# cvg/LightGlue

Hardware: AMD Instinct MI355X
Metric: image-pairs/s at N=M=1024, 9 layers; match-index parity vs ref (higher is better)
Workload: dtype f16; 1 GPU; SuperPoint-dim 256-d descriptors, N=M=1024, 9 layers, pruning/early-stop OFF, batch=32 pairs per GPU, seeded random weights (recipe A), precision=f16x3 (split-f16 operands, 3 MFMAs per product, for every contraction incl. q k^T and P V; fp32 accumulate / residual / softmax); pairs_per_gpu=32, keypoints=1024, keypoints1=1024, descriptor_dim=256, parallelism=pair-sharded dp1, batches_in_flight=1

## Files before the change

lightglue_amd/csrc/lg_assign.hip:

```cpp
#include "lg_kernels.h"

namespace lg {

__device__ __forceinline__ float fexp(float x) { return __builtin_amdgcn_exp2f(x * 1.44269504088896340736f); }

__device__ __forceinline__ void lse_merge(float& m, float& s, float m2, float s2) {
    const float mn = fmaxf(m, m2);
    if (mn == -INFINITY) { m = mn; s = 0.f; return; }
    s = s * fexp(m - mn) + s2 * fexp(m2 - mn);
    m = mn;
}

constexpr int ART = 32;

__device__ __forceinline__ void lse_merge1(float& m, float& s, float m2, float s2) {
    const float e = (m == m2) ? 1.f : fexp(-fabsf(m - m2));
    const bool keep = m >= m2;
    s = keep ? __builtin_fmaf(s2, e, s) : __builtin_fmaf(s, e, s2);
    m = keep ? m : m2;
}

__global__ __launch_bounds__(256) void lse_sweep_kernel(AssignArgs a) {
    const int pair = blockIdx.y, tile = blockIdx.x, tid = threadIdx.x, lane = tid & 63, wave = tid >> 6;
    const int len0 = a.rs.len[2 * pair], len1 = a.rs.len[2 * pair + 1];
    const int r0 = tile * ART;
    if (r0 >= len0) return;
    const int rows = min(ART, len0 - r0);
    const int ntiles = a.rs.cap0 / ART;
    const float* simp = a.sim + ((long long)pair * a.rs.cap0 + r0) * a.rs.cap1;
    float* pm = a.cpm + ((long long)pair * ntiles + tile) * a.rs.cap1;
    float* ps = a.cps + ((long long)pair * ntiles + tile) * a.rs.cap1;
    __shared__ float shm[4][ART], shs[4][ART];
    for (int c0 = 0; c0 < len1; c0 += 1024) {
        const int c = c0 + tid * 4;
        const bool act = c < len1;
        const float* col = simp + (act ? c : 0);
        float cm[4] = {-INFINITY, -INFINITY, -INFINITY, -INFINITY}, cs[4] = {0.f, 0.f, 0.f, 0.f};
        f32x4 nxt = *reinterpret_cast<const f32x4*>(col);
#pragma unroll 1
        for (int r = 0; r < rows; ++r) {
            f32x4 v = nxt;
            nxt = *reinterpret_cast<const f32x4*>(col + (long long)min(r + 1, rows - 1) * a.rs.cap1);
#pragma unroll
            for (int i = 0; i < 4; ++i) if (!act || c + i >= len1) v[i] = -INFINITY;
            const float m = wave_allmax(fmaxf(fmaxf(v[0], v[1]), fmaxf(v[2], v[3])));
            float sum = 0.f;
            if (m != -INFINITY) sum = (fexp(v[0] - m) + fexp(v[1] - m)) + (fexp(v[2] - m) + fexp(v[3] - m));
            if (act) {
#pragma unroll
                for (int i = 0; i < 4; ++i) lse_merge1(cm[i], cs[i], v[i], v[i] == -INFINITY ? 0.f : 1.f);
            }
            sum = wave_allsum(sum);
            if (lane == 0) {
                if (c0 == 0) { shm[wave][r] = m; shs[wave][r] = sum; }
                else { float mo = shm[wave][r], so = shs[wave][r]; lse_merge1(mo, so, m, sum); shm[wave][r] = mo; shs[wave][r] = so; }
            }
        }
        if (act) {
            *reinterpret_cast<f32x4*>(pm + c) = f32x4{cm[0], cm[1], cm[2], cm[3]};
            *reinterpret_cast<f32x4*>(ps + c) = f32x4{cs[0], cs[1], cs[2], cs[3]};
        }
    }
    __syncthreads();
    if (tid < rows) {
        float m = shm[0][tid], s = shs[0][tid];
        for (int w = 1; w < 4; ++w) lse_merge1(m, s, shm[w][tid], shs[w][tid]);
        a.lse_r[(long long)pair * a.rs.cap0 + r0 + tid] = m + logf(s);
    }
}

__global__ __launch_bounds__(256) void col_lse_merge_kernel(AssignArgs a) {
    const int pair = blockIdx.y, lane = threadIdx.x & 63, wave = threadIdx.x >> 6, c = blockIdx.x * 64 + lane;
    const int len0 = a.rs.len[2 * pair], len1 = a.rs.len[2 * pair + 1];
    if (blockIdx.x * 64 >= len1) return;
    const int ntiles = a.rs.cap0 / ART, live = (len0 + ART - 1) / ART;
    const int cc = min(c, a.rs.cap1 - 1);
    const float* pm = a.cpm + (long long)pair * ntiles * a.rs.cap1 + cc;
    const float* ps = a.cps + (long long)pair * ntiles * a.rs.cap1 + cc;
    float m = -INFINITY, s = 0.f;
#pragma unroll 8
    for (int t = wave; t < live; t += 4) lse_merge1(m, s, pm[(long long)t * a.rs.cap1], ps[(long long)t * a.rs.cap1]);
    __shared__ float shm[4][64], shs[4][64];
    shm[wave][lane] = m; shs[wave][lane] = s;
    __syncthreads();
    if (wave == 0 && c < len1) {
#pragma unroll
        for (int w = 1; w < 4; ++w) lse_merge1(m, s, shm[w][lane], shs[w][lane]);
        a.lse_c[(long long)pair * a.rs.cap1 + c] = m + logf(s);
    }
}

__device__ __forceinline__ float score_of(float sim, float lr, float lc, float cert) {
    return ((sim - lr) + (sim - lc)) + cert;
}

__global__ __launch_bounds__(256) void argmax_sweep_kernel(AssignArgs a) {
    const int pair = blockIdx.y, tile = blockIdx.x, tid = threadIdx.x, lane = tid & 63, wave = tid >> 6;
    const int len0 = a.rs.len[2 * pair], len1 = a.rs.len[2 * pair + 1];
    const int r0 = tile * ART;
    if (r0 >= len0) return;
    const int rows = min(ART, len0 - r0);
    const int ntiles = a.rs.cap0 / ART;
    const float* simp = a.sim + ((long long)pair * a.rs.cap0 + r0) * a.rs.cap1;
    const float* lsec = a.lse_c + (long long)pair * a.rs.cap1;
    const float* ls1 = a.ls + seg_row_base(a.rs, 2 * pair + 1);
    const float* lser = a.lse_r + (long long)pair * a.rs.cap0 + r0;
    const float* ls0 = a.ls + seg_row_base(a.rs, 2 * pair) + r0;
    float* pv = a.cbv + ((long long)pair * ntiles + tile) * a.rs.cap1;
    int* pi = a.cbi + ((long long)pair * ntiles + tile) * a.rs.cap1;
    __shared__ float shb[4][ART]; __shared__ int shi[4][ART];
    for (int c0 = 0; c0 < len1; c0 += 1024) {
        const int c = c0 + tid * 4;
        const bool act = c < len1;
        const int cc = act ? c : 0;
        const float* col = simp + cc;
        const f32x4 lc = *reinterpret_cast<const f32x4*>(lsec + cc);
        const f32x4 l1 = *reinterpret_cast<const f32x4*>(ls1 + cc);
        float cb[4] = {-INFINITY, -INFINITY, -INFINITY, -INFINITY}; int ci[4] = {0, 0, 0, 0};
        f32x4 nxt = *reinterpret_cast<const f32x4*>(col);
#pragma unroll 1
        for (int r = 0; r < rows; ++r) {
            const f32x4 v = nxt;
            nxt = *reinterpret_cast<const f32x4*>(col + (long long)min(r + 1, rows - 1) * a.rs.cap1);
            const float lr = lser[r], l0 = ls0[r];
            float best = -INFINITY; int bi = 0x7fffffff;
#pragma unroll
            for (int i = 0; i < 4; ++i) {
                if (act && c + i < len1) {
                    const float sc = score_of(v[i], lr, lc[i], l0 + l1[i]);
                    if (sc > best) { best = sc; bi = c + i; }
                    if (sc > cb[i]) { cb[i] = sc; ci[i] = r0 + r; }
                }
            }
            const float wbest = wave_allmax(best);
            const unsigned long long owners = __ballot(best == wbest);
            const int wbi = __builtin_amdgcn_readlane(bi, (int)__builtin_ctzll(owners));
            if (lane == 0) {
                if (c0 == 0 || wbest > shb[wave][r]) { shb[wave][r] = wbest; shi[wave][r] = wbi; }
            }
        }
        if (act) {
            *reinterpret_cast<f32x4*>(pv + c) = f32x4{cb[0], cb[1], cb[2], cb[3]};
            *reinterpret_cast<int4*>(pi + c) = int4{ci[0], ci[1], ci[2], ci[3]};
        }
    }
    __syncthreads();
    if (tid < rows) {
        float best = shb[0][tid]; int bi = shi[0][tid];
        for (int w = 1; w < 4; ++w) {
            const float ob = shb[w][tid]; const int oi = shi[w][tid];
            if (ob > best || (ob == best && oi < bi)) { best = ob; bi = oi; }
        }
        a.max0[(long long)pair * a.rs.cap0 + r0 + tid] = best; a.arg0[(long long)pair * a.rs.cap0 + r0 + tid] = bi;
    }
}

__global__ __launch_bounds__(256) void col_argmax_merge_kernel(AssignArgs a) {
    const int pair = blockIdx.y, lane = threadIdx.x & 63, wave = threadIdx.x >> 6, c = blockIdx.x * 64 + lane;
    const int len0 = a.rs.len[2 * pair], len1 = a.rs.len[2 * pair + 1];
    if (blockIdx.x * 64 >= len1) return;
    const int ntiles = a.rs.cap0 / ART, live = (len0 + ART - 1) / ART;
    const int cc = min(c, a.rs.cap1 - 1);
    const float* pv = a.cbv + (long long)pair * ntiles * a.rs.cap1 + cc;
    const int* pi = a.cbi + (long long)pair * ntiles * a.rs.cap1 + cc;
    float best = -INFINITY; int bi = 0;
#pragma unroll 8
    for (int t = wave; t < live; t += 4) {
        const float v = pv[(long long)t * a.rs.cap1];
        const int vi = pi[(long long)t * a.rs.cap1];
        if (v > best) { best = v; bi = vi; }
    }
    __shared__ float shb[4][64]; __shared__ int shi[4][64];
    shb[wave][lane] = best; shi[wave][lane] = bi;
    __syncthreads();
    if (wave == 0 && c < len1) {
#pragma unroll
        for (int w = 1; w < 4; ++w) {
            const float v = shb[w][lane]; const int vi = shi[w][lane];
            if (v > best || (v == best && v != -INFINITY && vi < bi)) { best = v; bi = vi; }
        }
        a.max1[(long long)pair * a.rs.cap1 + c] = best; a.arg1[(long long)pair * a.rs.cap1 + c] = bi;
    }
}

struct Row0 { bool valid; int j; float e; };
__device__ __forceinline__ Row0 match_of_row0(const AssignArgs& a, const float* max0, const int* arg0, const int* arg1, int r, int len1) {
    const int jraw = arg0[r];
    const bool jok = (unsigned)jraw < (unsigned)len1;
    const int j = jok ? jraw : 0;
    const bool mutual0 = jok && arg1[j] == r;
    const float e = mutual0 ? expf(max0[r]) : 0.f;
    return {mutual0 && (e > a.filter_threshold), j, e};
}
__global__ __launch_bounds__(256) void finalize_kernel(AssignArgs a) {
    const int pair = blockIdx.y, blk = blockIdx.x, tid = threadIdx.x, lane = tid & 63, wave = tid >> 6;
    const int len0 = a.rs.len[2 * pair], len1 = a.rs.len[2 * pair + 1];
    const int base0 = seg_row_base(a.rs, 2 * pair), base1 = seg_row_base(a.rs, 2 * pair + 1);
    const float* max0 = a.max0 + (long long)pair * a.rs.cap0;
    const int* arg0 = a.arg0 + (long long)pair * a.rs.cap0;
    const int* arg1 = a.arg1 + (long long)pair * a.rs.cap1;
    int* m0 = a.m0 + (long long)pair * a.n0; float* s0 = a.s0 + (long long)pair * a.n0;
    int* m1 = a.m1 + (long long)pair * a.n1; float* s1 = a.s1 + (long long)pair * a.n1;
    __shared__ int sh_cnt[4], sh_below[4];
    if (len0 == 0 || len1 == 0) { if (blk == 0 && tid == 0) a.n_matches[pair] = 0; return; }
    {
        const int b = blk * 256 + tid;
        if (b < len1) {
            const int i = arg1[b];
            const bool mutual1 = arg0[i] == b;
            const float e = expf(max0[i]);
            const bool valid1 = mutual1 && (e > a.filter_threshold);
            const int ob = a.ind[base1 + b];
            m1[ob] = valid1 ? a.ind[base0 + i] : -1;
            s1[ob] = mutual1 ? e : 0.f;
        }
    }
    if (blk * 256 >= len0 && blk != (int)gridDim.x - 1) return;
    int below = 0;
    for (int q = 0; q < blk; ++q) {
        const int r = q * 256 + tid;
        below += __popcll(__ballot(r < len0 && match_of_row0(a, max0, arg0, arg1, min(r, len0 - 1), len1).valid));
    }
    const int r = blk * 256 + tid;
    bool valid0 = false; int oa = 0, ob = -1; float e = 0.f;
    if (r < len0) {
        const Row0 m = match_of_row0(a, max0, arg0, arg1, r, len1);
        valid0 = m.valid; e = m.e;
        oa = a.ind[base0 + r];
        ob = valid0 ? a.ind[base1 + m.j] : -1;
        m0[oa] = ob;
        s0[oa] = e;
    }
    const unsigned long long bal = __ballot(valid0);
    const int prefix = __popcll(bal & ((1ull << lane) - 1ull));
    if (lane == 0) { sh_cnt[wave] = __popcll(bal); sh_below[wave] = below; }
    __syncthreads();
    int woff = sh_below[0] + sh_below[1] + sh_below[2] + sh_below[3];
    for (int w = 0; w < wave; ++w) woff += sh_cnt[w];
    if (valid0) {
        int* ml = a.matches + (long long)pair * a.max_matches * 2;
        float* msl = a.mscores + (long long)pair * a.max_matches;
        const int k = woff + prefix;
        ml[2 * k] = oa; ml[2 * k + 1] = ob; msl[k] = e;
    }
    if (blk == (int)gridDim.x - 1 && tid == 0)
        a.n_matches[pair] = sh_below[0] + sh_below[1] + sh_below[2] + sh_below[3] + sh_cnt[0] + sh_cnt[1] + sh_cnt[2] + sh_cnt[3];
}

__global__ __launch_bounds__(256) void fill_neg_inf_kernel(float* p, long long n) {
    for (long long i = (long long)blockIdx.x * 256 + threadIdx.x; i < n; i += (long long)gridDim.x * 256) p[i] = -INFINITY;
}
__global__ __launch_bounds__(256) void log_assignment_kernel(AssignArgs a) {
    const int pair = blockIdx.y, r = blockIdx.x, tid = threadIdx.x;
    const int len0 = a.rs.len[2 * pair], len1 = a.rs.len[2 * pair + 1];
    const int base0 = seg_row_base(a.rs, 2 * pair), base1 = seg_row_base(a.rs, 2 * pair + 1);
    float* out = a.log_assignment + (long long)pair * (a.n0 + 1) * (a.n1 + 1);
    if (len0 == 0 || len1 == 0) {
        if (r == a.rs.cap0 && tid == 0) out[(long long)a.n0 * (a.n1 + 1) + a.n1] = 0.f;
        return;
    }
    if (r == a.rs.cap0) {
        for (int c = tid; c < len1; c += 256) out[(long long)a.n0 * (a.n1 + 1) + a.ind[base1 + c]] = a.lsneg[base1 + c];
        if (tid == 0) out[(long long)a.n0 * (a.n1 + 1) + a.n1] = 0.f;
        return;
    }
    if (r >= len0) return;
    float* orow = out + (long long)a.ind[base0 + r] * (a.n1 + 1);
    const float* simr = a.sim + ((long long)pair * a.rs.cap0 + r) * a.rs.cap1;
    const float lr = a.lse_r[(long long)pair * a.rs.cap0 + r], l0 = a.ls[base0 + r];
    const float* lsec = a.lse_c + (long long)pair * a.rs.cap1;
    for (int c = tid; c < len1; c += 256) orow[a.ind[base1 + c]] = score_of(simr[c], lr, lsec[c], l0 + a.ls[base1 + c]);
    if (tid == 0) orow[a.n1] = a.lsneg[base0 + r];
}

hipError_t launch_assign(const AssignArgs& a, hipStream_t s) {
    const int B = a.rs.B;
    hipError_t e;
    if (!a.all_rows_live) {
    if (a.n0 > 0) {
        if ((e = hipMemsetAsync(a.m0, 0xFF, sizeof(int) * (size_t)B * a.n0, s)) != hipSuccess) return e;
        if ((e = hipMemsetAsync(a.s0, 0, sizeof(float) * (size_t)B * a.n0, s)) != hipSuccess) return e;
    }
    if (a.n1 > 0) {
        if ((e = hipMemsetAsync(a.m1, 0xFF, sizeof(int) * (size_t)B * a.n1, s)) != hipSuccess) return e;
        if ((e = hipMemsetAsync(a.s1, 0, sizeof(float) * (size_t)B * a.n1, s)) != hipSuccess) return e;
    }
    }
    hipLaunchKernelGGL(lse_sweep_kernel, dim3(a.rs.cap0 / ART, B), dim3(256), 0, s, a);
    hipLaunchKernelGGL(col_lse_merge_kernel, dim3(a.rs.cap1 / 64, B), dim3(256), 0, s, a);
    hipLaunchKernelGGL(argmax_sweep_kernel, dim3(a.rs.cap0 / ART, B), dim3(256), 0, s, a);
    hipLaunchKernelGGL(col_argmax_merge_kernel, dim3(a.rs.cap1 / 64, B), dim3(256), 0, s, a);
    hipLaunchKernelGGL(finalize_kernel, dim3((max(a.rs.cap0, a.rs.cap1) + 255) / 256, B), dim3(256), 0, s, a);
    if (a.log_assignment) {
        const long long total = (long long)B * (a.n0 + 1) * (a.n1 + 1);
        hipLaunchKernelGGL(fill_neg_inf_kernel, dim3(2048), dim3(256), 0, s, a.log_assignment, total);
        hipLaunchKernelGGL(log_assignment_kernel, dim3(a.rs.cap0 + 1, B), dim3(256), 0, s, a);
    }
    return hipGetLastError();
}

}
```

lightglue_amd/csrc/lg_proj.hip:

```cpp
#include "lg_proj_body.h"
#include "lg_side.h"

namespace lg {

__device__ __forceinline__ bool proj_tile(const RowSpace& rs, TileLoc& t, int& len) {
    t = locate_tile(rs, blockIdx.x, PBM);
    len = rs.len[t.seg];
    if (t.r0 >= len) return false;
    if (rs.active && !rs.active[t.pair]) return false;
    return true;
}
__device__ __forceinline__ bool proj_tile(const RowSpace& rs, TileLoc& t) { int len; return proj_tile(rs, t, len); }

template <int PREC> struct TileRegs {
    static constexpr int NV = PJ<PREC>::Tag::EPC / 4, KE = PJL<PREC>::KE, STAGES = PJL<PREC>::STAGES;
    f32x4 v[STAGES][NV];
    __device__ __forceinline__ void load(const float* src) {
#pragma unroll
        for (int st = 0; st < STAGES; ++st)
#pragma unroll
            for (int j = 0; j < NV; ++j) v[st][j] = *reinterpret_cast<const f32x4*>(src + st * KE + 4 * j);
    }
    __device__ __forceinline__ void load_f16(const f16_t* src) {
#pragma unroll
        for (int st = 0; st < STAGES; ++st) {
            if constexpr (NV == 2) {
                const f16x8 h = *reinterpret_cast<const f16x8*>(src + st * KE);
                v[st][0] = widen4_f16(h.lo); v[st][1] = widen4_f16(h.hi);
            } else {
                static_assert(NV == 1, "4 or 8 elements per chunk");
                v[st][0] = widen4_f16(*reinterpret_cast<const f16x4*>(src + st * KE));
            }
        }
    }
    __device__ __forceinline__ void store(char* smA, int srow, int sslot, bool copy_out, float* xdst) const {
        const int off = pj_tile_off(srow, sslot);
#pragma unroll
        for (int st = 0; st < STAGES; ++st) {
            if (copy_out) {
#pragma unroll
                for (int j = 0; j < NV; ++j) *reinterpret_cast<f32x4*>(xdst + st * KE + 4 * j) = v[st][j];
            }
            char* tile = smA + st * PJL<PREC>::TILE;
            if constexpr (PREC == PREC_F32) {
                *reinterpret_cast<f32x4*>(tile + off) = v[st][0];
            } else if constexpr (PJ<PREC>::APART == 2) {
                u32x4 hi, lo;
                split8<typename PJ<PREC>::Tag>(v[st][0], v[st][1], hi, lo);
                *reinterpret_cast<u32x4*>(tile + off) = hi;
                *reinterpret_cast<u32x4*>(tile + PJL<PREC>::A_PLANE + off) = lo;
            } else {
                *reinterpret_cast<u32x4*>(tile + off) = pack8<typename PJ<PREC>::Tag>(v[st][0], v[st][1]);
            }
        }
    }
};
template <int PREC>
__device__ __forceinline__ void proj_load_tile(const float* X, const TileLoc& t, char* smA) {
    const int srow = threadIdx.x >> 3, sslot = threadIdx.x & 7;
    TileRegs<PREC> h;
    h.load(X + (long long)(t.grow0 + srow) * 256 + sslot * PJ<PREC>::Tag::EPC);
    h.store(smA, srow, sslot, false, nullptr);
}

template <int PREC, class TA, int NTP, int NPASS>
__global__ __launch_bounds__(PTHREADS) void proj_kernel(ProjArgs a) {
    extern __shared__ __attribute__((aligned(16))) char smem[];
    char* smA = smem;

    TileLoc t;
    if (!proj_tile(a.rs, t)) return;
    const int tid = threadIdx.x, lane = tid & 63, w = __builtin_amdgcn_readfirstlane(tid >> 6);
    if (a.dbg && lane == 0) dbg_slot(a.dbg, w, 0) = clock64();
    RopeRows<4> rr;
    if constexpr (NTP == 3) proj_rope_load<4>(a, t, rr);
    proj_load_tile<PREC>(a.X, t, smA);
    proj_compute<PREC, TA, NTP, NPASS>(a, t, smA, 0, NTP == 3 ? &rr : nullptr);
}

struct RowDest { float* X; float* cosb; float* sinb; };

struct FirstRows {
    typedef PrepArgs Args;
    const PrepArgs& pa;
    const PrepSide& sd;
    int seg; long long simg, in_row;
    __device__ __forceinline__ FirstRows(const PrepArgs& pa_, const TileLoc& t, int rc) : pa(pa_), sd(pa_.side[t.seg & 1]), seg(t.seg) {
        simg = source_image(pa.px, t.pair, seg & 1);
        in_row = simg * sd.n + rc;
    }
    template <int PREC> __device__ __forceinline__ void load_x(TileRegs<PREC>& h, int col) const {
        if (sd.kind == DESC_F16) h.load_f16(static_cast<const f16_t*>(sd.desc) + in_row * 256 + col);
        else h.load(static_cast<const float*>(sd.desc) + in_row * 256 + col);
    }
    __device__ __forceinline__ void rotary(int sslot, f32x4& c4, f32x4& s4) const {
        float kn[4];
        normalised_keypoint(pa, sd, seg, simg, in_row, kn);
#pragma unroll
        for (int f = 0; f < 4; ++f) {
            const float p = fourier_phase(pa, kn, sslot * 4 + f);
            c4[f] = cosf(p); s4[f] = sinf(p);
        }
    }
    __device__ __forceinline__ RowDest dest() const { return {pa.X, pa.cosb, pa.sinb}; }
    __device__ __forceinline__ void row_stored(long long grow, int r, int sslot) const { if (sslot == 0) pa.ind[grow] = r; }
};
struct GatherRows {
    typedef GatherArgs Args;
    const GatherArgs& ga;
    long long in_row;
    __device__ __forceinline__ GatherRows(const GatherArgs& ga_, const TileLoc& t, int rc) : ga(ga_) {
        const long long base = t.grow0 - t.r0;
        const int sr = ga.len_old[t.seg] >= 0 ? ga.src[base + rc] : rc;
        in_row = base + sr;
    }
    template <int PREC> __device__ __forceinline__ void load_x(TileRegs<PREC>& h, int col) const { h.load(ga.Xold + in_row * 256 + col); }
    __device__ __forceinline__ void rotary(int sslot, f32x4& c4, f32x4& s4) const {
        c4 = *reinterpret_cast<const f32x4*>(ga.cos_old + in_row * 32 + sslot * 4);
        s4 = *reinterpret_cast<const f32x4*>(ga.sin_old + in_row * 32 + sslot * 4);
    }
    __device__ __forceinline__ RowDest dest() const { return {ga.Xnew, ga.cos_new, ga.sin_new}; }
    __device__ __forceinline__ void row_stored(long long, int, int) const {}
};

template <int PREC, class TA, class Rows>
__global__ __launch_bounds__(PTHREADS) void proj_rows_kernel(ProjArgs a, typename Rows::Args sa) {
    constexpr int EPC = PJ<PREC>::Tag::EPC;
    extern __shared__ __attribute__((aligned(16))) char smem[];
    char* smA = smem;
    float* ldsC = reinterpret_cast<float*>(smem + PJL<PREC>::A_BYTES);
    float* ldsS = ldsC + PBM * 32;

    TileLoc t;
    int len;
    if (!proj_tile(a.rs, t, len)) return;
    const int tid = threadIdx.x, lane = tid & 63, w = __builtin_amdgcn_readfirstlane(tid >> 6), lr = lane & 15, g = lane >> 4;
    const int srow = tid >> 3, sslot = tid & 7;
    const int r = t.r0 + srow, rc = r < len ? r : len - 1;
    const Rows rows(sa, t, rc);
    const RowDest dst = rows.dest();
    TileRegs<PREC> h;
    rows.load_x(h, sslot * EPC);
    {
        f32x4 c4, s4;
        rows.rotary(sslot, c4, s4);
        *reinterpret_cast<f32x4*>(ldsC + srow * 32 + sslot * 4) = c4;
        *reinterpret_cast<f32x4*>(ldsS + srow * 32 + sslot * 4) = s4;
        if (r < len) {
            const long long grow = t.grow0 + srow;
            *reinterpret_cast<f32x4*>(dst.cosb + grow * 32 + sslot * 4) = c4;
            *reinterpret_cast<f32x4*>(dst.sinb + grow * 32 + sslot * 4) = s4;
            rows.row_stored(grow, r, sslot);
        }
    }
    h.store(smA, srow, sslot, r < len, dst.X + (long long)(t.grow0 + srow) * 256 + sslot * EPC);
    __syncthreads();
    RopeRows<4> rr;
    {
        const int f0 = ((32 * w) & 63) / 2 + 4 * g;
#pragma unroll
        for (int mt = 0; mt < 4; ++mt) {
            const int row = pj_row<4>(mt, lr);
            rr.c[mt] = *reinterpret_cast<const f32x4*>(ldsC + row * 32 + f0);
            rr.s[mt] = *reinterpret_cast<const f32x4*>(ldsS + row * 32 + f0);
        }
    }
    proj_compute<PREC, TA, 3, 2>(a, t, smA, 0, &rr);
}
template <class Rows> static hipError_t launch_proj_rows(int prec, int attn_prec, const ProjArgs& a, const typename Rows::Args& sa, hipStream_t s) {
    return dispatch_qkv_prec(prec, attn_prec, a.plane, [&](auto P, auto ta) {
        constexpr int PREC = decltype(P)::value;
        const int R = a.rs.B * (a.rs.cap0 + a.rs.cap1);
        return launch_with_lds(proj_rows_kernel<PREC, decltype(ta), Rows>, dim3(R / PBM), dim3(PTHREADS), PJL<PREC>::A_BYTES + 2 * PBM * 32 * 4, s, a, sa);
    });
}
hipError_t launch_proj_first(int prec, int attn_prec, const ProjArgs& a, const PrepArgs& pa, hipStream_t s) {
    if (!(a.Nout == 768 && a.n_qk_groups == 2 && a.cosb && a.sinb) || pa.input_dim != 256) return hipErrorInvalidValue;
    return launch_proj_rows<FirstRows>(prec, attn_prec, a, pa, s);
}
hipError_t launch_proj_gather(int prec, int attn_prec, const ProjArgs& a, const GatherArgs& g, hipStream_t s) {
    if (!(a.Nout == 768 && a.n_qk_groups == 2) || !g.Xold || !g.Xnew || !g.src || !g.len_old) return hipErrorInvalidValue;
    return launch_proj_rows<GatherRows>(prec, attn_prec, a, g, s);
}

template <int PREC>
__global__ __launch_bounds__(PTHREADS) void final_proj_kernel(FinalArgs a) {
    extern __shared__ __attribute__((aligned(16))) char smem[];
    TileLoc t;
    if (!proj_tile(a.rs, t)) return;
    proj_load_tile<PREC>((a.xsel && a.xsel[t.pair]) ? a.X2 : a.X, t, smem);
    final_compute<PREC>(a, t, smem);
}
template <int PREC> static hipError_t launch_final_t(const FinalArgs& a, hipStream_t s) {
    return launch_with_lds(final_proj_kernel<PREC>, dim3(a.R / PBM), dim3(PTHREADS), PJL<PREC>::A_BYTES, s, a);
}
hipError_t launch_final_proj(int prec, const FinalArgs& a, hipStream_t s) {
    switch (prec) {
        case PREC_F32: return launch_final_t<PREC_F32>(a, s);
        case PREC_BF16: return launch_final_t<PREC_BF16>(a, s);
        case PREC_F16: return launch_final_t<PREC_F16>(a, s);
        case PREC_F16X3: return launch_final_t<PREC_F16X3>(a, s);
    }
    return hipErrorInvalidValue;
}

template <int PREC, class TA, int NTP, int NPASS> static hipError_t launch_proj_t(const ProjArgs& a, hipStream_t s) {
    const int R = a.rs.B * (a.rs.cap0 + a.rs.cap1);
    return launch_with_lds(proj_kernel<PREC, TA, NTP, NPASS>, dim3(R / PBM), dim3(PTHREADS), PJL<PREC>::A_BYTES, s, a);
}
hipError_t launch_proj(int prec, int attn_prec, const ProjArgs& a, hipStream_t s) {
    return dispatch_qkv_prec(prec, attn_prec, a.plane, [&](auto P, auto ta) {
        constexpr int PREC = decltype(P)::value;
        typedef decltype(ta) TA;
        if (a.Nout == 768 && a.n_qk_groups == 2 && a.cosb && a.sinb) return launch_proj_t<PREC, TA, 3, 2>(a, s);
        if (a.Nout == 512 && a.n_qk_groups == 1) return launch_proj_t<PREC, TA, 2, 2>(a, s);
        return hipErrorInvalidValue;
    });
}

}
```

lightglue_amd/csrc/lg_proj_body.h:

```cpp
#pragma once
#include <type_traits>

#include "lg_kernels.h"

namespace lg {

constexpr int PBM = 64, PTHREADS = 512;
constexpr float QK_PRESCALE = 0.42466090014400953f;

constexpr int PREC_QKV_F16W2 = 100;
template <int PREC> struct PJ;
template <> struct PJ<PREC_F32> { typedef TagF32 Tag; static constexpr int NPART = 1, APART = 1, OPART = 1; };
template <> struct PJ<PREC_BF16> { typedef TagBF16 Tag; static constexpr int NPART = 1, APART = 1, OPART = 1; };
template <> struct PJ<PREC_F16> { typedef TagF16 Tag; static constexpr int NPART = 1, APART = 1, OPART = 1; };
template <> struct PJ<PREC_F16X3> { typedef TagF16 Tag; static constexpr int NPART = 2, APART = 2, OPART = 2; };
template <> struct PJ<PREC_QKV_F16W2> { typedef TagF16 Tag; static constexpr int NPART = 2, APART = 1, OPART = 1; };

template <class F> hipError_t dispatch_qkv_prec(int prec, int attn_prec, long long plane, F f) {
    if (prec == PREC_F32 && attn_prec == PREC_F32) return f(std::integral_constant<int, PREC_F32>{}, float());
    if (prec == PREC_BF16 && attn_prec == PREC_BF16) return f(std::integral_constant<int, PREC_BF16>{}, bf16_t());
    if (prec == PREC_F16 && attn_prec == PREC_F16) return f(std::integral_constant<int, PREC_F16>{}, f16_t());
    if (prec == PREC_F16X3 && attn_prec == PREC_F16X3) return plane > 0 ? f(std::integral_constant<int, PREC_F16X3>{}, f16_t()) : hipErrorInvalidValue;
    if (prec == PREC_F16X3 && attn_prec == PREC_F16) return f(std::integral_constant<int, PREC_QKV_F16W2>{}, f16_t());
    return hipErrorInvalidValue;
}

template <int PREC, bool TRANSPOSED>
__device__ __forceinline__ void pj_mma(f32x4& acc, const u32x4* wf, const u32x4* xf) {
    typedef typename PJ<PREC>::Tag Tag;
    auto mm = [&](const u32x4& wv, const u32x4& xv) { if constexpr (TRANSPOSED) mma_chunk<Tag>(acc, wv, xv); else mma_chunk<Tag>(acc, xv, wv); };
    if constexpr (PJ<PREC>::NPART == 2 && PJ<PREC>::APART == 2) { mm(wf[0], xf[1]); mm(wf[1], xf[0]); mm(wf[0], xf[0]); }
    else if constexpr (PJ<PREC>::NPART == 2) { mm(wf[1], xf[0]); mm(wf[0], xf[0]); }
    else mm(wf[0], xf[0]);
}

template <class T> __device__ __forceinline__ T pj_cvt(float x);
template <> __device__ __forceinline__ float pj_cvt<float>(float x) { return x; }
template <> __device__ __forceinline__ bf16_t pj_cvt<bf16_t>(float x) { return (bf16_t)x; }
template <> __device__ __forceinline__ f16_t pj_cvt<f16_t>(float x) { return (f16_t)x; }

template <int PREC> struct PJL {
    typedef typename PJ<PREC>::Tag Tag;
    static constexpr int KE = 8 * Tag::EPC;
    static constexpr int STAGES = 256 / KE;
    static constexpr int TILE = PBM * 128;
    static constexpr int A_PLANE = STAGES * TILE;
    static constexpr int A_BYTES = PJ<PREC>::APART * A_PLANE;
};
template <int MT> __device__ __forceinline__ int pj_row(int mt, int slot) {
    if constexpr (MT >= 2) return 32 * (mt >> 1) + 8 * (slot >> 2) + 4 * (mt & 1) + (slot & 3);
    else return slot;
}
__device__ __forceinline__ int pj_tile_off(int row, int slot16) { return row * 128 + ((slot16 ^ (((row >> 1) & 1) | (((row >> 3) & 3) << 1))) << 4); }
template <int NTP> __device__ __forceinline__ constexpr bool pj_is_v(int pass, int j) { return NTP == 3 ? j == 2 : pass == 1; }
template <int NTP> __device__ __forceinline__ int pj_tile(int w, int pass, int j) {
    if constexpr (NTP == 3) return j < 2 ? 16 * pass + 2 * w + j : 32 + w + 8 * pass;
    else return pass == 0 ? 2 * w + j : 16 + w + 8 * j;
}
template <int NKC> __device__ __forceinline__ u32x4 packed_weight_frag(__amdgpu_buffer_rsrc_t rsrc, int lane16, int p, int plane_bytes, int nt, int kc) {
    return weight_frag(rsrc, lane16, (p ? plane_bytes : 0) + (nt * NKC + kc) * 1024);
}
template <class Tag> __device__ __forceinline__ int proj_plane_bytes(const ProjArgs& a) { return a.Nout * 256 * (int)sizeof(typename Tag::elem); }
template <int PREC, class TA>
__device__ __forceinline__ void store8_qkv(TA* dst, long long plane, const f32x4& v0, const f32x4& v1) {
    if constexpr (PJ<PREC>::OPART == 2) {
        u32x4 hi, lo;
        split8_f16<true>(v0, v1, hi, lo);
        *reinterpret_cast<u32x4*>(dst) = hi;
        *reinterpret_cast<u32x4*>(dst + plane) = lo;
    } else if constexpr (sizeof(TA) == 2) {
        *reinterpret_cast<u32x4*>(dst) = pack8<typename PJ<PREC>::Tag>(v0, v1);
    } else {
        *reinterpret_cast<f32x4*>(dst) = v0; *reinterpret_cast<f32x4*>(dst + 4) = v1;
    }
}
template <class T> __device__ __forceinline__ void store4_split(T* dst, long long plane, const f32x4& v) {
    uint32_t h01, l01, h23, l23;
    split2_f16(v[0], v[1], h01, l01); split2_f16(v[2], v[3], h23, l23);
    *reinterpret_cast<u32x2*>(dst) = u32x2{h01, h23};
    *reinterpret_cast<u32x2*>(dst + plane) = u32x2{l01, l23};
}

template <int MT> struct RopeRows { f32x4 c[MT], s[MT]; };
template <int MT>
__device__ __forceinline__ void proj_rope_load(const ProjArgs& a, const TileLoc& t, RopeRows<MT>& rr) {
    const int tid = threadIdx.x, lane = tid & 63, w = __builtin_amdgcn_readfirstlane(tid >> 6), lr = lane & 15, g = lane >> 4;
    const int pcol = 32 * w;
#pragma unroll
    for (int mt = 0; mt < MT; ++mt) {
        const long long row = t.grow0 + pj_row<MT>(mt, lr);
        rr.c[mt] = *reinterpret_cast<const f32x4*>(a.cosb + row * 32 + ((pcol & 63) >> 1) + 4 * g);
        rr.s[mt] = *reinterpret_cast<const f32x4*>(a.sinb + row * 32 + ((pcol & 63) >> 1) + 4 * g);
    }
}
template <int PREC, class TA, int NTP, int NPASS, int PASS, int A_PLANE, int MT, bool AHEAD>
__device__ __forceinline__ void proj_pass(const ProjArgs& a, const TileLoc& t, const char* smA, u32x4 (&bf)[PJ<PREC>::NPART == 2 ? 2 : 4][NTP][PJ<PREC>::NPART],
                                          int stamp_base, const RopeRows<MT>& rr) {
    typedef typename PJ<PREC>::Tag Tag;
    constexpr int NPART = PJ<PREC>::NPART, APART = PJ<PREC>::APART;
    constexpr int STAGES = PJL<PREC>::STAGES, NKC = 2 * STAGES, TILE = MT * 16 * 128;
    constexpr int NBUF = NPART == 2 ? 2 : 4;
    const int tid = threadIdx.x, lane = tid & 63, w = __builtin_amdgcn_readfirstlane(tid >> 6), lr = lane & 15, g = lane >> 4;
    const long long R = a.R;
    auto stamp = [&](int slot) {
        if (a.dbg && lane == 0) dbg_slot(a.dbg, w, stamp_base + slot) = clock64();
    };
    const __amdgpu_buffer_rsrc_t wrs = weight_rsrc(a.W);
    const int lane16 = lane * 16;
    auto load_b = [&](u32x4 (&dst)[NTP][NPART], int pass, int kc) {
#pragma unroll
        for (int j = 0; j < NTP; ++j)
#pragma unroll
            for (int p = 0; p < NPART; ++p) dst[j][p] = packed_weight_frag<NKC>(wrs, lane16, p, proj_plane_bytes<Tag>(a), pj_tile<NTP>(w, pass, j), kc);
    };
    constexpr bool HAS_PAIR = !pj_is_v<NTP>(PASS, 0);
    constexpr bool ROPE = NTP == 3;
    const int pcol = (NTP == 3 ? PASS * 256 : 0) + 32 * w;
    f32x4 pb[2]; f32x4 pc[MT], ps[MT]; float bv[NTP];
    auto load_operands = [&]() {
        if constexpr (HAS_PAIR) {
            pb[0] = *reinterpret_cast<const f32x4*>(a.bias + pcol + 8 * g); pb[1] = *reinterpret_cast<const f32x4*>(a.bias + pcol + 8 * g + 4);
            if constexpr (ROPE) {
#pragma unroll
                for (int mt = 0; mt < MT; ++mt) { pc[mt] = rr.c[mt]; ps[mt] = rr.s[mt]; }
            }
        }
#pragma unroll
        for (int j = 0; j < NTP; ++j)
            if (pj_is_v<NTP>(PASS, j)) bv[j] = a.bias[pj_tile<NTP>(w, PASS, j) * 16 + lr];
    };
    if constexpr (AHEAD) load_operands();
    f32x4 acc[MT][NTP];
#pragma unroll
    for (int i = 0; i < MT; ++i)
#pragma unroll
        for (int j = 0; j < NTP; ++j) acc[i][j] = f32x4{0.f, 0.f, 0.f, 0.f};
    static_assert(MT <= 4 && NBUF % 2 == 0, "row tiles per workgroup / ring depth");
    u32x4 afh[2][MT][APART];
    auto read_af = [&](u32x4 (&af)[MT][APART], int kc) {
        const char* tile = smA + (kc >> 1) * TILE;
#pragma unroll
        for (int mt = 0; mt < MT; ++mt)
#pragma unroll
            for (int p = 0; p < APART; ++p)
                af[mt][p] = *reinterpret_cast<const u32x4*>(tile + p * A_PLANE + pj_tile_off(pj_row<MT>(mt, lr), (kc & 1) * 4 + g));
    };
    if constexpr (AHEAD) read_af(afh[0], 0);
#pragma unroll 1
    for (int c0 = 0; c0 < NKC; c0 += NBUF) {
#pragma unroll
        for (int i = 0; i < NBUF; ++i) {
            const int kc = c0 + i;
            const int nk = kc + NBUF - 1;
            const int npass = nk < NKC ? PASS : (PASS + 1 < NPASS ? PASS + 1 : PASS);
            load_b(bf[(i + NBUF - 1) % NBUF], npass, nk < NKC ? nk : nk - NKC);
            if constexpr (AHEAD) read_af(afh[(i + 1) & 1], kc + 1 < NKC ? kc + 1 : kc);
            __builtin_amdgcn_sched_barrier(0);
            if constexpr (!AHEAD) read_af(afh[i & 1], kc);
#pragma unroll
            for (int mt = 0; mt < MT; ++mt)
#pragma unroll
                for (int j = 0; j < NTP; ++j) {
                    if (pj_is_v<NTP>(PASS, j)) pj_mma<PREC, false>(acc[mt][j], bf[i][j], afh[i & 1][mt]);
                    else pj_mma<PREC, true>(acc[mt][j], bf[i][j], afh[i & 1][mt]);
                }
            __builtin_amdgcn_sched_barrier(0);
        }
    }
    stamp(2 + 2 * PASS);
    if constexpr (!AHEAD) load_operands();
    typedef TA ta4 __attribute__((ext_vector_type(4)));
    const bool range_on = a.range_flag != nullptr;
    const int live_rows = range_on ? a.rs.len[t.seg] - t.r0 : 0;
    bool out_of_range = false;
    constexpr int OPART = PJ<PREC>::OPART;
    static_assert(OPART == 1 || sizeof(TA) == 2, "split q / k / v planes are f16");
    if constexpr (HAS_PAIR) {
        TA* base = static_cast<TA*>((NTP == 3 && PASS == 1) ? a.k : a.q);
        const int head = (pcol >> 6) & 3, d0 = pcol & 63;
#pragma unroll
        for (int mt = 0; mt < MT; ++mt) {
            const long long row = t.grow0 + pj_row<MT>(mt, lr);
            f32x4 v0 = acc[mt][0] + pb[0], v1 = acc[mt][1] + pb[1];
            if constexpr (ROPE) {
                const f32x4 c = pc[mt], sn = ps[mt];
                const f32x4 u0 = v0, u1 = v1;
                v0[0] = u0[0] * c[0] - u0[1] * sn[0]; v0[1] = u0[1] * c[0] + u0[0] * sn[0];
                v0[2] = u0[2] * c[1] - u0[3] * sn[1]; v0[3] = u0[3] * c[1] + u0[2] * sn[1];
                v1[0] = u1[0] * c[2] - u1[1] * sn[2]; v1[1] = u1[1] * c[2] + u1[0] * sn[2];
                v1[2] = u1[2] * c[3] - u1[3] * sn[3]; v1[3] = u1[3] * c[3] + u1[2] * sn[3];
            }
            v0 *= QK_PRESCALE; v1 *= QK_PRESCALE;
            if (range_on && pj_row<MT>(mt, lr) < live_rows) out_of_range |= out_of_f16_range(v0) | out_of_f16_range(v1);
            TA* dst = base + ((long long)head * R + row) * 64 + d0 + 8 * g;
            store8_qkv<PREC>(dst, a.plane, v0, v1);
        }
    }
#pragma unroll
    for (int j = 0; j < NTP; ++j) {
        if (!pj_is_v<NTP>(PASS, j)) continue;
        const int col0 = pj_tile<NTP>(w, PASS, j) * 16;
        const int head = (col0 >> 6) & 3, d0 = col0 & 63;
        TA* vrow = static_cast<TA*>(a.vt) + ((long long)head * 64 + d0 + lr) * R + t.grow0;
        if constexpr (MT >= 2) {
#pragma unroll
            for (int q = 0; q < MT / 2; ++q) {
                const f32x4 v0 = acc[2 * q][j] + bv[j], v1 = acc[2 * q + 1][j] + bv[j];
                TA* dst = vrow + 32 * q + 8 * g;
                if (range_on) {
#pragma unroll
                    for (int r = 0; r < 4; ++r) {
                        out_of_range |= (32 * q + 8 * g + r < live_rows) & out_of_f16_range(v0[r]);
                        out_of_range |= (32 * q + 8 * g + 4 + r < live_rows) & out_of_f16_range(v1[r]);
                    }
                }
                store8_qkv<PREC>(dst, a.plane, v0, v1);
            }
        } else {
            const f32x4 v = acc[0][j] + bv[j];
            TA* dst = vrow + 4 * g;
            if (range_on) {
#pragma unroll
                for (int r = 0; r < 4; ++r) out_of_range |= (4 * g + r < live_rows) & out_of_f16_range(v[r]);
            }
            if constexpr (OPART == 2) {
                store4_split(dst, a.plane, v);
            } else {
                ta4 o = {pj_cvt<TA>(v[0]), pj_cvt<TA>(v[1]), pj_cvt<TA>(v[2]), pj_cvt<TA>(v[3])};
                *reinterpret_cast<ta4*>(dst) = o;
            }
        }
    }
    if (range_on && out_of_range) a.range_flag[t.pair] = 1;
    stamp(3 + 2 * PASS);
}

template <int PREC, class TA, int NTP, int NPASS, int A_PLANE = PJL<PREC>::A_PLANE, int MT = 4, bool AHEAD = false>
__device__ __forceinline__ void proj_compute(const ProjArgs& a, const TileLoc& t, const char* smA, int stamp_base, const RopeRows<MT>* preloaded = nullptr) {
    static_assert(NPASS == 2, "two passes");
    typedef typename PJ<PREC>::Tag Tag;
    constexpr int NPART = PJ<PREC>::NPART;
    constexpr int NKC = 2 * PJL<PREC>::STAGES;
    constexpr int NBUF = NPART == 2 ? 2 : 4;
    const int tid = threadIdx.x, lane = tid & 63, w = __builtin_amdgcn_readfirstlane(tid >> 6);
    u32x4 bf[NBUF][NTP][NPART];
#pragma unroll
    for (int i = 0; i < NBUF - 1; ++i)
#pragma unroll
        for (int j = 0; j < NTP; ++j)
#pragma unroll
            for (int p = 0; p < NPART; ++p) bf[i][j][p] = packed_weight_frag<NKC>(weight_rsrc(a.W), lane * 16, p, proj_plane_bytes<Tag>(a), pj_tile<NTP>(w, 0, j), i);
    RopeRows<MT> rr;
    if constexpr (NTP == 3) { if (preloaded) rr = *preloaded; else proj_rope_load<MT>(a, t, rr); }
    __syncthreads();
    if (a.dbg && lane == 0) dbg_slot(a.dbg, w, stamp_base + 1) = clock64();
    proj_pass<PREC, TA, NTP, NPASS, 0, A_PLANE, MT, AHEAD>(a, t, smA, bf, stamp_base, rr);
    proj_pass<PREC, TA, NTP, NPASS, 1, A_PLANE, MT, AHEAD>(a, t, smA, bf, stamp_base, rr);
}

template <int PREC, int A_PLANE = PJL<PREC>::A_PLANE, int MT = 4>
__device__ __forceinline__ void final_compute(const FinalArgs& a, const TileLoc& t, const char* smA) {
    typedef typename PJ<PREC>::Tag Tag;
    constexpr int NPART = PJ<PREC>::NPART, APART = PJ<PREC>::APART;
    constexpr int STAGES = PJL<PREC>::STAGES, NKC = 2 * STAGES, TILE = MT * 16 * 128;
    constexpr int NBUF = 4;
    const int tid = threadIdx.x, lane = tid & 63, w = __builtin_amdgcn_readfirstlane(tid >> 6), lr = lane & 15, g = lane >> 4;
    const int layer = a.layer_of_pair ? a.layer_of_pair[t.pair] : 0;
    const __amdgpu_buffer_rsrc_t wrs = weight_rsrc(static_cast<const char*>(a.W) + (long long)layer * a.w_layer_bytes);
    const float* bias = a.bias + (long long)layer * 256;
    const int lane16 = lane * 16;
    constexpr int plane_bytes = 256 * 256 * (int)sizeof(typename Tag::elem);
    auto load_b = [&](u32x4 (&dst)[2][NPART], int kc) {
#pragma unroll
        for (int j = 0; j < 2; ++j)
#pragma unroll
            for (int p = 0; p < NPART; ++p) dst[j][p] = packed_weight_frag<NKC>(wrs, lane16, p, plane_bytes, 2 * w + j, kc);
    };
    u32x4 bf[NBUF][2][NPART];
#pragma unroll
    for (int i = 0; i < NBUF - 1; ++i) load_b(bf[i], i);
    f32x4 b4[2];
#pragma unroll
    for (int j = 0; j < 2; ++j) b4[j] = *reinterpret_cast<const f32x4*>(bias + (2 * w + j) * 16 + 4 * g);
    __syncthreads();
    f32x4 acc[MT][2];
#pragma unroll
    for (int i = 0; i < MT; ++i) { acc[i][0] = f32x4{0.f, 0.f, 0.f, 0.f}; acc[i][1] = f32x4{0.f, 0.f, 0.f, 0.f}; }
#pragma unroll 1
    for (int c0 = 0; c0 < NKC; c0 += NBUF) {
#pragma unroll
        for (int i = 0; i < NBUF; ++i) {
            const int kc = c0 + i;
            load_b(bf[(i + NBUF - 1) % NBUF], kc + NBUF - 1 < NKC ? kc + NBUF - 1 : NKC - 1);
            __builtin_amdgcn_sched_barrier(0);
            const char* tile = smA + (kc >> 1) * TILE;
            u32x4 af[MT][APART];
#pragma unroll
            for (int mt = 0; mt < MT; ++mt)
#pragma unroll
                for (int p = 0; p < APART; ++p)
                    af[mt][p] = *reinterpret_cast<const u32x4*>(tile + p * A_PLANE + pj_tile_off(pj_row<MT>(mt, lr), (kc & 1) * 4 + g));
#pragma unroll
            for (int mt = 0; mt < MT; ++mt)
#pragma unroll
                for (int j = 0; j < 2; ++j) pj_mma<PREC, true>(acc[mt][j], bf[i][j], af[mt]);
            __builtin_amdgcn_sched_barrier(0);
        }
    }
    if constexpr (NPART == 2) {
        if (a.planes) {
            f16_t* md = reinterpret_cast<f16_t*>(a.out);
            const long long plane = (long long)a.R * 256;
#pragma unroll
            for (int mt = 0; mt < MT; ++mt) {
                f16_t* dst = md + (t.grow0 + pj_row<MT>(mt, lr)) * 256LL + 32 * w + 4 * g;
#pragma unroll
                for (int j = 0; j < 2; ++j) {
                    const f32x4 v = (acc[mt][j] + b4[j]) * a.scale;
                    store4_split(dst + 16 * j, plane, v);
                }
            }
            return;
        }
    }
#pragma unroll
    for (int mt = 0; mt < MT; ++mt) {
        float* dst = a.out + (t.grow0 + pj_row<MT>(mt, lr)) * 256LL + 32 * w + 4 * g;
#pragma unroll
        for (int j = 0; j < 2; ++j) *reinterpret_cast<f32x4*>(dst + 16 * j) = (acc[mt][j] + b4[j]) * a.scale;
    }
}

}
```

Before: 4284 image-pairs/s.

## Restructure self-attn QKV projection into three passes and deepen assign sweep prefetch

```diff
diff --git a/lightglue_amd/csrc/lg_assign.hip b/lightglue_amd/csrc/lg_assign.hip
--- a/lightglue_amd/csrc/lg_assign.hip
+++ b/lightglue_amd/csrc/lg_assign.hip
@@ -12,6 +12,25 @@
 }
 
 constexpr int ART = 32;
+
+constexpr int SWEEP_RING = 4;
+template <class F> __device__ __forceinline__ void sweep_rows(const float* col, int cap1, int rows, F row) {
+    f32x4 ring[SWEEP_RING];
+#pragma unroll
+    for (int i = 0; i < SWEEP_RING; ++i) ring[i] = *reinterpret_cast<const f32x4*>(col + (long long)min(i, rows - 1) * cap1);
+    int r = 0;
+#pragma unroll 1
+    for (; r + SWEEP_RING <= rows; r += SWEEP_RING) {
+#pragma unroll
+        for (int i = 0; i < SWEEP_RING; ++i) {
+            row(r + i, ring[i]);
+            ring[i] = *reinterpret_cast<const f32x4*>(col + (long long)min(r + i + SWEEP_RING, rows - 1) * cap1);
+        }
+    }
+#pragma unroll
+    for (int i = 0; i < SWEEP_RING - 1; ++i)
+        if (r + i < rows) row(r + i, ring[i]);
+}
 
 __device__ __forceinline__ void lse_merge1(float& m, float& s, float m2, float s2) {
     const float e = (m == m2) ? 1.f : fexp(-fabsf(m - m2));
@@ -36,11 +55,7 @@
         const bool act = c < len1;
         const float* col = simp + (act ? c : 0);
         float cm[4] = {-INFINITY, -INFINITY, -INFINITY, -INFINITY}, cs[4] = {0.f, 0.f, 0.f, 0.f};
-        f32x4 nxt = *reinterpret_cast<const f32x4*>(col);
-#pragma unroll 1
-        for (int r = 0; r < rows; ++r) {
-            f32x4 v = nxt;
-            nxt = *reinterpret_cast<const f32x4*>(col + (long long)min(r + 1, rows - 1) * a.rs.cap1);
+        auto row = [&](int r, f32x4 v) {
 #pragma unroll
             for (int i = 0; i < 4; ++i) if (!act || c + i >= len1) v[i] = -INFINITY;
             const float m = wave_allmax(fmaxf(fmaxf(v[0], v[1]), fmaxf(v[2], v[3])));
@@ -55,7 +70,8 @@
                 if (c0 == 0) { shm[wave][r] = m; shs[wave][r] = sum; }
                 else { float mo = shm[wave][r], so = shs[wave][r]; lse_merge1(mo, so, m, sum); shm[wave][r] = mo; shs[wave][r] = so; }
             }
-        }
+        };
+        sweep_rows(col, a.rs.cap1, rows, row);
         if (act) {
             *reinterpret_cast<f32x4*>(pm + c) = f32x4{cm[0], cm[1], cm[2], cm[3]};
             *reinterpret_cast<f32x4*>(ps + c) = f32x4{cs[0], cs[1], cs[2], cs[3]};
@@ -109,6 +125,7 @@
     float* pv = a.cbv + ((long long)pair * ntiles + tile) * a.rs.cap1;
     int* pi = a.cbi + ((long long)pair * ntiles + tile) * a.rs.cap1;
     __shared__ float shb[4][ART]; __shared__ int shi[4][ART];
+    const float lser_l = lser[min(lane, rows - 1)], ls0_l = ls0[min(lane, rows - 1)];
     for (int c0 = 0; c0 < len1; c0 += 1024) {
         const int c = c0 + tid * 4;
         const bool act = c < len1;
@@ -117,12 +134,9 @@
         const f32x4 lc = *reinterpret_cast<const f32x4*>(lsec + cc);
         const f32x4 l1 = *reinterpret_cast<const f32x4*>(ls1 + cc);
         float cb[4] = {-INFINITY, -INFINITY, -INFINITY, -INFINITY}; int ci[4] = {0, 0, 0, 0};
-        f32x4 nxt = *reinterpret_cast<const f32x4*>(col);
-#pragma unroll 1
-        for (int r = 0; r < rows; ++r) {
-            const f32x4 v = nxt;
-            nxt = *reinterpret_cast<const f32x4*>(col + (long long)min(r + 1, rows - 1) * a.rs.cap1);
-            const float lr = lser[r], l0 = ls0[r];
+        auto row = [&](int r, const f32x4 v) {
+            const float lr = __int_as_float(__builtin_amdgcn_readlane(__float_as_int(lser_l), r));
+            const float l0 = __int_as_float(__builtin_amdgcn_readlane(__float_as_int(ls0_l), r));
             float best = -INFINITY; int bi = 0x7fffffff;
 #pragma unroll
             for (int i = 0; i < 4; ++i) {
@@ -138,7 +152,8 @@
             if (lane == 0) {
                 if (c0 == 0 || wbest > shb[wave][r]) { shb[wave][r] = wbest; shi[wave][r] = wbi; }
             }
-        }
+        };
+        sweep_rows(col, a.rs.cap1, rows, row);
         if (act) {
             *reinterpret_cast<f32x4*>(pv + c) = f32x4{cb[0], cb[1], cb[2], cb[3]};
             *reinterpret_cast<int4*>(pi + c) = int4{ci[0], ci[1], ci[2], ci[3]};
diff --git a/lightglue_amd/csrc/lg_proj.hip b/lightglue_amd/csrc/lg_proj.hip
--- a/lightglue_amd/csrc/lg_proj.hip
+++ b/lightglue_amd/csrc/lg_proj.hip
@@ -63,8 +63,9 @@
     h.store(smA, srow, sslot, false, nullptr);
 }
 
+constexpr int PROJ_WAVES = 2 * PTHREADS / 256;
 template <int PREC, class TA, int NTP, int NPASS>
-__global__ __launch_bounds__(PTHREADS) void proj_kernel(ProjArgs a) {
+__global__ __launch_bounds__(PTHREADS, PROJ_WAVES) void proj_kernel(ProjArgs a) {
     extern __shared__ __attribute__((aligned(16))) char smem[];
     char* smA = smem;
 
@@ -73,9 +74,9 @@
     const int tid = threadIdx.x, lane = tid & 63, w = __builtin_amdgcn_readfirstlane(tid >> 6);
     if (a.dbg && lane == 0) dbg_slot(a.dbg, w, 0) = clock64();
     RopeRows<4> rr;
-    if constexpr (NTP == 3) proj_rope_load<4>(a, t, rr);
+    if constexpr (pj_self<NTP, NPASS>) proj_rope_load<4>(a, t, rr);
     proj_load_tile<PREC>(a.X, t, smA);
-    proj_compute<PREC, TA, NTP, NPASS>(a, t, smA, 0, NTP == 3 ? &rr : nullptr);
+    proj_compute<PREC, TA, NTP, NPASS>(a, t, smA, 0, pj_self<NTP, NPASS> ? &rr : nullptr);
 }
 
 struct RowDest { float* X; float* cosb; float* sinb; };
@@ -124,11 +125,12 @@
 };
 
 template <int PREC, class TA, class Rows>
-__global__ __launch_bounds__(PTHREADS) void proj_rows_kernel(ProjArgs a, typename Rows::Args sa) {
+__global__ __launch_bounds__(PTHREADS, PROJ_WAVES) void proj_rows_kernel(ProjArgs a, typename Rows::Args sa) {
     constexpr int EPC = PJ<PREC>::Tag::EPC;
     extern __shared__ __attribute__((aligned(16))) char smem[];
     char* smA = smem;
-    float* ldsC = reinterpret_cast<float*>(smem + PJL<PREC>::A_BYTES);
+    static_assert(2 * PBM * 32 * 4 <= PJL<PREC>::A_BYTES, "the rotary rows fit the activation tile");
+    float* ldsC = reinterpret_cast<float*>(smem);
     float* ldsS = ldsC + PBM * 32;
 
     TileLoc t;
@@ -153,7 +155,6 @@
             rows.row_stored(grow, r, sslot);
         }
     }
-    h.store(smA, srow, sslot, r < len, dst.X + (long long)(t.grow0 + srow) * 256 + sslot * EPC);
     __syncthreads();
     RopeRows<4> rr;
     {
@@ -165,13 +166,15 @@
             rr.s[mt] = *reinterpret_cast<const f32x4*>(ldsS + row * 32 + f0);
         }
     }
-    proj_compute<PREC, TA, 3, 2>(a, t, smA, 0, &rr);
+    __syncthreads();
+    h.store(smA, srow, sslot, r < len, dst.X + (long long)(t.grow0 + srow) * 256 + sslot * EPC);
+    proj_compute<PREC, TA, 2, 3>(a, t, smA, 0, &rr);
 }
 template <class Rows> static hipError_t launch_proj_rows(int prec, int attn_prec, const ProjArgs& a, const typename Rows::Args& sa, hipStream_t s) {
     return dispatch_qkv_prec(prec, attn_prec, a.plane, [&](auto P, auto ta) {
         constexpr int PREC = decltype(P)::value;
         const int R = a.rs.B * (a.rs.cap0 + a.rs.cap1);
-        return launch_with_lds(proj_rows_kernel<PREC, decltype(ta), Rows>, dim3(R / PBM), dim3(PTHREADS), PJL<PREC>::A_BYTES + 2 * PBM * 32 * 4, s, a, sa);
+        return launch_with_lds(proj_rows_kernel<PREC, decltype(ta), Rows>, dim3(R / PBM), dim3(PTHREADS), PJL<PREC>::A_BYTES, s, a, sa);
     });
 }
 hipError_t launch_proj_first(int prec, int attn_prec, const ProjArgs& a, const PrepArgs& pa, hipStream_t s) {
@@ -212,7 +215,7 @@
     return dispatch_qkv_prec(prec, attn_prec, a.plane, [&](auto P, auto ta) {
         constexpr int PREC = decltype(P)::value;
         typedef decltype(ta) TA;
-        if (a.Nout == 768 && a.n_qk_groups == 2 && a.cosb && a.sinb) return launch_proj_t<PREC, TA, 3, 2>(a, s);
+        if (a.Nout == 768 && a.n_qk_groups == 2 && a.cosb && a.sinb) return launch_proj_t<PREC, TA, 2, 3>(a, s);
         if (a.Nout == 512 && a.n_qk_groups == 1) return launch_proj_t<PREC, TA, 2, 2>(a, s);
         return hipErrorInvalidValue;
     });
diff --git a/lightglue_amd/csrc/lg_proj_body.h b/lightglue_amd/csrc/lg_proj_body.h
--- a/lightglue_amd/csrc/lg_proj_body.h
+++ b/lightglue_amd/csrc/lg_proj_body.h
@@ -52,9 +52,14 @@
     else return slot;
 }
 __device__ __forceinline__ int pj_tile_off(int row, int slot16) { return row * 128 + ((slot16 ^ (((row >> 1) & 1) | (((row >> 3) & 3) << 1))) << 4); }
-template <int NTP> __device__ __forceinline__ constexpr bool pj_is_v(int pass, int j) { return NTP == 3 ? j == 2 : pass == 1; }
-template <int NTP> __device__ __forceinline__ int pj_tile(int w, int pass, int j) {
-    if constexpr (NTP == 3) return j < 2 ? 16 * pass + 2 * w + j : 32 + w + 8 * pass;
+template <int NTP, int NPASS> constexpr bool pj_self = NTP * NPASS == 6;
+template <int NTP, int NPASS> __device__ __forceinline__ constexpr bool pj_is_v(int pass, int j) {
+    static_assert((NTP == 3 && NPASS == 2) || (NTP == 2 && (NPASS == 2 || NPASS == 3)), "self 3 x 2 or 2 x 3, cross 2 x 2");
+    return NPASS == 3 ? pass == 2 : (NTP == 3 ? j == 2 : pass == 1);
+}
+template <int NTP, int NPASS> __device__ __forceinline__ int pj_tile(int w, int pass, int j) {
+    if constexpr (NPASS == 3) return pass < 2 ? 16 * pass + 2 * w + j : 32 + w + 8 * j;
+    else if constexpr (NTP == 3) return j < 2 ? 16 * pass + 2 * w + j : 32 + w + 8 * pass;
     else return pass == 0 ? 2 * w + j : 16 + w + 8 * j;
 }
 template <int NKC> __device__ __forceinline__ u32x4 packed_weight_frag(__amdgpu_buffer_rsrc_t rsrc, int lane16, int p, int plane_bytes, int nt, int kc) {
@@ -111,11 +116,11 @@
 #pragma unroll
         for (int j = 0; j < NTP; ++j)
 #pragma unroll
-            for (int p = 0; p < NPART; ++p) dst[j][p] = packed_weight_frag<NKC>(wrs, lane16, p, proj_plane_bytes<Tag>(a), pj_tile<NTP>(w, pass, j), kc);
-    };
-    constexpr bool HAS_PAIR = !pj_is_v<NTP>(PASS, 0);
-    constexpr bool ROPE = NTP == 3;
-    const int pcol = (NTP == 3 ? PASS * 256 : 0) + 32 * w;
+            for (int p = 0; p < NPART; ++p) dst[j][p] = packed_weight_frag<NKC>(wrs, lane16, p, proj_plane_bytes<Tag>(a), pj_tile<NTP, NPASS>(w, pass, j), kc);
+    };
+    constexpr bool HAS_PAIR = !pj_is_v<NTP, NPASS>(PASS, 0);
+    constexpr bool ROPE = pj_self<NTP, NPASS>;
+    const int pcol = (pj_self<NTP, NPASS> ? PASS * 256 : 0) + 32 * w;
     f32x4 pb[2]; f32x4 pc[MT], ps[MT]; float bv[NTP];
     auto load_operands = [&]() {
         if constexpr (HAS_PAIR) {
@@ -127,7 +132,7 @@
         }
 #pragma unroll
         for (int j = 0; j < NTP; ++j)
-            if (pj_is_v<NTP>(PASS, j)) bv[j] = a.bias[pj_tile<NTP>(w, PASS, j) * 16 + lr];
+            if (pj_is_v<NTP, NPASS>(PASS, j)) bv[j] = a.bias[pj_tile<NTP, NPASS>(w, PASS, j) * 16 + lr];
     };
     if constexpr (AHEAD) load_operands();
     f32x4 acc[MT][NTP];
@@ -161,7 +166,7 @@
             for (int mt = 0; mt < MT; ++mt)
 #pragma unroll
                 for (int j = 0; j < NTP; ++j) {
-                    if (pj_is_v<NTP>(PASS, j)) pj_mma<PREC, false>(acc[mt][j], bf[i][j], afh[i & 1][mt]);
+                    if (pj_is_v<NTP, NPASS>(PASS, j)) pj_mma<PREC, false>(acc[mt][j], bf[i][j], afh[i & 1][mt]);
                     else pj_mma<PREC, true>(acc[mt][j], bf[i][j], afh[i & 1][mt]);
                 }
             __builtin_amdgcn_sched_barrier(0);
@@ -176,7 +181,7 @@
     constexpr int OPART = PJ<PREC>::OPART;
     static_assert(OPART == 1 || sizeof(TA) == 2, "split q / k / v planes are f16");
     if constexpr (HAS_PAIR) {
-        TA* base = static_cast<TA*>((NTP == 3 && PASS == 1) ? a.k : a.q);
+        TA* base = static_cast<TA*>((pj_self<NTP, NPASS> && PASS == 1) ? a.k : a.q);
         const int head = (pcol >> 6) & 3, d0 = pcol & 63;
 #pragma unroll
         for (int mt = 0; mt < MT; ++mt) {
@@ -191,15 +196,18 @@
                 v1[2] = u1[2] * c[3] - u1[3] * sn[3]; v1[3] = u1[3] * c[3] + u1[2] * sn[3];
             }
             v0 *= QK_PRESCALE; v1 *= QK_PRESCALE;
-            if (range_on && pj_row<MT>(mt, lr) < live_rows) out_of_range |= out_of_f16_range(v0) | out_of_f16_range(v1);
+            bool live;
+            if constexpr (NPASS == 3) live = pj_row<MT>(0, lr) < live_rows - pj_row<MT>(mt, 0);
+            else live = pj_row<MT>(mt, lr) < live_rows;
+            if (range_on && live) out_of_range |= out_of_f16_range(v0) | out_of_f16_range(v1);
             TA* dst = base + ((long long)head * R + row) * 64 + d0 + 8 * g;
             store8_qkv<PREC>(dst, a.plane, v0, v1);
         }
     }
 #pragma unroll
     for (int j = 0; j < NTP; ++j) {
-        if (!pj_is_v<NTP>(PASS, j)) continue;
-        const int col0 = pj_tile<NTP>(w, PASS, j) * 16;
+        if (!pj_is_v<NTP, NPASS>(PASS, j)) continue;
+        const int col0 = pj_tile<NTP, NPASS>(w, PASS, j) * 16;
         const int head = (col0 >> 6) & 3, d0 = col0 & 63;
         TA* vrow = static_cast<TA*>(a.vt) + ((long long)head * 64 + d0 + lr) * R + t.grow0;
         if constexpr (MT >= 2) {
@@ -237,7 +245,6 @@
 
 template <int PREC, class TA, int NTP, int NPASS, int A_PLANE = PJL<PREC>::A_PLANE, int MT = 4, bool AHEAD = false>
 __device__ __forceinline__ void proj_compute(const ProjArgs& a, const TileLoc& t, const char* smA, int stamp_base, const RopeRows<MT>* preloaded = nullptr) {
-    static_assert(NPASS == 2, "two passes");
     typedef typename PJ<PREC>::Tag Tag;
     constexpr int NPART = PJ<PREC>::NPART;
     constexpr int NKC = 2 * PJL<PREC>::STAGES;
@@ -249,13 +256,14 @@
 #pragma unroll
         for (int j = 0; j < NTP; ++j)
 #pragma unroll
-            for (int p = 0; p < NPART; ++p) bf[i][j][p] = packed_weight_frag<NKC>(weight_rsrc(a.W), lane * 16, p, proj_plane_bytes<Tag>(a), pj_tile<NTP>(w, 0, j), i);
+            for (int p = 0; p < NPART; ++p) bf[i][j][p] = packed_weight_frag<NKC>(weight_rsrc(a.W), lane * 16, p, proj_plane_bytes<Tag>(a), pj_tile<NTP, NPASS>(w, 0, j), i);
     RopeRows<MT> rr;
-    if constexpr (NTP == 3) { if (preloaded) rr = *preloaded; else proj_rope_load<MT>(a, t, rr); }
+    if constexpr (pj_self<NTP, NPASS>) { if (preloaded) rr = *preloaded; else proj_rope_load<MT>(a, t, rr); }
     __syncthreads();
     if (a.dbg && lane == 0) dbg_slot(a.dbg, w, stamp_base + 1) = clock64();
     proj_pass<PREC, TA, NTP, NPASS, 0, A_PLANE, MT, AHEAD>(a, t, smA, bf, stamp_base, rr);
     proj_pass<PREC, TA, NTP, NPASS, 1, A_PLANE, MT, AHEAD>(a, t, smA, bf, stamp_base, rr);
+    if constexpr (NPASS == 3) proj_pass<PREC, TA, NTP, NPASS, 2, A_PLANE, MT, AHEAD>(a, t, smA, bf, stamp_base, rr);
 }
 
 template <int PREC, int A_PLANE = PJL<PREC>::A_PLANE, int MT = 4>
```

Result: no change. 4293 image-pairs/s, median of 6 (+0.2%).
